# RDG0818/MAZero

Hardware: NVIDIA B200
Metric: mcts_sims_per_sec (higher is better)
Workload: dtype bf16

## Files before the change

### mazero_b200/csrc/search_persist.cuh

```cuda
#pragma once
#include "infer_hmma.cuh"
#include "tree_step.cuh"

namespace maz {
namespace persist {

using namespace hmma;

struct SearchParams {
    Desc d;
    TreeLayout L;
    char *arena;
    const float *lam_pow, *logterm;
    const double *sqrtn;
    int table_len;
    float discount;
    int K, S;
    int *g_err;
    int *idx_y;
    int *greedy_w;
    float *rec_r, *rec_v, *rec_p, *rec_b;
    int *rec_ix, *rec_act;
    long long *tree_clock;
};

__device__ __forceinline__ unsigned long long globaltimer_ns()
{
    unsigned long long t;
    asm volatile("mov.u64 %0, %globaltimer;" : "=l"(t));
    return t;
}

constexpr uint32_t TREE_SCRATCH_OFF = OFF_PH;
constexpr uint32_t TREE_SCRATCH_BYTES = OFF_STAT - OFF_PH;

struct ExtraMap {
    uint32_t hot_stride;
    uint32_t o_qd, o_path, o_exp, o_dep;
    uint32_t o_xr, o_xv, o_xp, o_xb, o_xi, o_xa;
    uint32_t bytes;
};
__host__ __device__ inline uint32_t al16(uint32_t x) { return (x + 15u) & ~15u; }
__host__ __device__ inline ExtraMap extra_map(int rpt, int Nt, int A, int S)
{
    ExtraMap m;
    const uint32_t lv = (uint32_t)S + 2;
    m.o_qd = 64;
    m.o_path = m.o_qd + al16(4 * lv);
    m.o_exp = m.o_path + al16(2 * lv);
    m.o_dep = m.o_exp + al16(2 * lv);
    m.hot_stride = m.o_dep + al16(2 * lv);
    uint32_t o = m.hot_stride * (uint32_t)rpt;
    const uint32_t NA = (uint32_t)Nt * A;
    m.o_xr = o; o += al16(4 * rpt);
    m.o_xv = o; o += al16(4 * rpt);
    m.o_xp = o; o += al16(4 * rpt * NA);
    m.o_xb = o; o += al16(4 * rpt * NA);
    m.o_xi = o; o += al16(4 * rpt);
    m.o_xa = o; o += al16(4 * rpt * Nt);
    m.bytes = o;
    return m;
}
__host__ __device__ inline size_t persist_smem_bytes(int vec_floats, int rpt, int Nt, int A, int S)
{
    return ((smem_bytes(vec_floats) + 15) & ~(size_t)15) + extra_map(rpt, Nt, A, S).bytes;
}

__device__ __forceinline__ void gather_root(const Desc &d, int root, int rl, int ix, const int *tree_act, int lane)
{
    HSM_DECL;
    const int N = d.N;
#pragma unroll 1
    for (int j0 = 0; j0 < N; j0 += 4) {
        float4 v[4];
        int act[4];
#pragma unroll
        for (int u = 0; u < 4; ++u) {
            const int j = j0 + u;
            if (j < N) {
                v[u] = __ldcg(reinterpret_cast<const float4 *>(d.pool + ((size_t)ix * d.B + root) * (size_t)(N * H) + (size_t)j * H) + lane);
                if (d.greedy_pool == nullptr || d.cur < 0) act[u] = tree_act[j];
                else if (j == d.cur) act[u] = tree_act[0];
                else if (j < d.cur) act[u] = d.factor ? __ldcg(d.factor + (size_t)root * N + j) : 0;
                else act[u] = __ldcg(d.greedy_pool + ((size_t)ix * d.B + root) * N + j);
            }
        }
#pragma unroll
        for (int u = 0; u < 4; ++u) {
            const int j = j0 + u;
            if (j < N) {
                const int r = rl * N + j;
                *reinterpret_cast<uint2 *>(hsm + OFF_HH + (size_t)r * LDA + lane * 8) = make_uint2(pack2(v[u].x, v[u].y), pack2(v[u].z, v[u].w));
                if (2 * lane < d.KA)
                    *reinterpret_cast<uint32_t *>(hsm + OFF_ONE + (size_t)r * LDO + lane * 4) =
                        pack2((2 * lane == act[u]) ? 1.f : 0.f, (2 * lane + 1 == act[u]) ? 1.f : 0.f);
            }
        }
    }
}

constexpr int PERSIST_THREADS = NCONS + 128;
constexpr int REGS_COMPUTE = 232, REGS_PRODUCER = 40;

template <bool kProf>
__global__ void __launch_bounds__(PERSIST_THREADS, 1) k_search_persistent(const __grid_constant__ SearchParams P)
{
    HSM_DECL;
    __shared__ __align__(8) uint64_t bar_full[NSLOT], bar_empty[NSLOT], bar_vec;
    const Desc &d = P.d;
    const int tid = threadIdx.x, warp = tid >> 5, lane = tid & 31;

    if (tid == 0) {
        for (int i = 0; i < NSLOT; ++i) { mbar_init(&bar_full[i], 1); mbar_init(&bar_empty[i], NCONS / 32); }
        mbar_init(&bar_vec, 1);
        mbar_fence_init();
    }
    setup_rows(d);
    for (uint32_t o = tid * 16u; o < TM * (uint32_t)LDA + TM * (uint32_t)LDO; o += PERSIST_THREADS * 16u)
        *reinterpret_cast<uint4 *>(hsm + OFF_HH + o) = make_uint4(0u, 0u, 0u, 0u);
    __syncthreads();
    if (warp >= NCONS / 32) {
        asm volatile("setmaxnreg.dec.sync.aligned.u32 %0;" ::"n"(REGS_PRODUCER));
        if (warp == NCONS / 32 && lane == 0) produce_weights(d, bar_full, bar_empty, &bar_vec, P.S);
        return;
    }
    asm volatile("setmaxnreg.inc.sync.aligned.u32 %0;" ::"n"(REGS_COMPUTE));
    Ring ring{bar_full, bar_empty, 0};
    TreeLayout Lprof = P.L;
    if (kProf && P.tree_clock != nullptr)
        Lprof.dbg_clock = P.tree_clock + 2 * P.S + 4 * (long long)gridDim.x + 64 + 4 * (long long)P.d.B;
    const TreeLayout &L = kProf ? Lprof : P.L;
    const int rpt = tile_rpt(d);
    const int root0 = blockIdx.x * rpt;
    const int tree = root0 + warp;
    const bool has_tree = warp < rpt && tree < d.B;
    char *tb = P.arena + (size_t)(has_tree ? tree : 0) * L.slab_bytes;
    const size_t B = (size_t)d.B, NA = (size_t)L.N * L.A;
    const StepScratch scr = carve_step_scratch(reinterpret_cast<char *>(hsm) + TREE_SCRATCH_OFF + (size_t)warp * tree_scratch_bytes(L.N, L.A, L.K, L.S),
                                               L.N, L.A, L.K, L.S);
    const ExtraMap xm = extra_map(rpt, L.N, L.A, L.S);
    char *xbase = reinterpret_cast<char *>(hsm) + ((smem_bytes(d.vec_floats) + 15) & ~(size_t)15);
    char *hb = xbase + (size_t)(warp < rpt ? warp : 0) * xm.hot_stride;
    TreeHdr *hdr = reinterpret_cast<TreeHdr *>(hb);
    const TreeHot hot{reinterpret_cast<uint16_t *>(hb + xm.o_path), reinterpret_cast<float *>(hb + xm.o_qd),
                      reinterpret_cast<uint16_t *>(hb + xm.o_exp), reinterpret_cast<uint16_t *>(hb + xm.o_dep)};
    float *x_r = reinterpret_cast<float *>(xbase + xm.o_xr), *x_v = reinterpret_cast<float *>(xbase + xm.o_xv);
    float *x_p = reinterpret_cast<float *>(xbase + xm.o_xp), *x_b = reinterpret_cast<float *>(xbase + xm.o_xb);
    int *x_i = reinterpret_cast<int *>(xbase + xm.o_xi), *x_a = reinterpret_cast<int *>(xbase + xm.o_xa);
    if (has_tree) {
        const TreeHot g = hot_from_slab(L, tb);
        if (lane < 16) reinterpret_cast<int *>(hdr)[lane] = reinterpret_cast<const int *>(f_hdr(tb))[lane];
        for (int i = lane; i < L.S + 2; i += 32) {
            hot.path[i] = g.path[i]; hot.qd[i] = g.qd[i]; hot.expslot[i] = g.expslot[i]; hot.depth[i] = g.depth[i];
        }
    }
    __syncwarp();

    long long *clk = (kProf && P.tree_clock != nullptr && blockIdx.x == 0 && tid == 0) ? P.tree_clock : nullptr;
    long long *cta_clk = (kProf && P.tree_clock != nullptr && tid == 0) ? P.tree_clock + 2 * P.S + 4 * blockIdx.x : nullptr;
    const long long k0 = cta_clk ? clock64() : 0;
    const unsigned long long g0 = cta_clk ? globaltimer_ns() : 0;
    long long sum_inf = 0, sum_tree = 0;
    long long *tree_clk = (kProf && P.tree_clock != nullptr && has_tree && lane == 0)
                              ? P.tree_clock + 2 * P.S + 4 * (long long)gridDim.x + 64 + 4 * (long long)tree : nullptr;
    long long tc_eb = 0, tc_sel = 0, tc_len = 0, tc_max = 0;

    mbar_wait(&bar_vec, 0);
    setup_head_copies(d);
    cta_sync();

    SimIo io;
    io.idx_x = x_i; io.actions = x_a; io.reward = x_r; io.value = x_v; io.probs = x_p; io.beta = x_b; io.root0 = root0;
    io.logits_out = nullptr;

#pragma unroll 1
    for (int s = 0; s <= P.S; ++s) {
        const long long t1 = cta_clk ? clock64() : 0;
        if (has_tree) {
            const long long q0 = tree_clk ? clock64() : 0;
            if (s > 0) {
                if (P.rec_r != nullptr) {
                    const size_t o = (size_t)(s - 1) * B + tree;
                    if (lane == 0) { P.rec_r[o] = x_r[warp]; P.rec_v[o] = x_v[warp]; }
                    for (int t = lane; t < (int)NA; t += 32) {
                        P.rec_p[o * NA + t] = x_p[(size_t)warp * NA + t];
                        P.rec_b[o * NA + t] = x_b[(size_t)warp * NA + t];
                    }
                }
                expand_backup_device<false>(L, tb, hdr, hot, P.lam_pow, s, P.discount, P.K, x_r + warp, x_v + warp, x_p + (size_t)warp * NA,
                                            x_b + (size_t)warp * NA, scr, lane, P.g_err, kProf ? tree : -1);
            }
            __syncwarp();
            if (kProf && s > 0 && L.dbg_clock != nullptr && tree == 0 && lane == 0) {
                const int order[11] = {0, 1, 2, 11, 12, 13, 14, 15, 3, 4, 5};
                for (int i = 1; i < 11; ++i) L.dbg_clock[16 + i] += L.dbg_clock[order[i]] - L.dbg_clock[order[i - 1]];
            }
            const long long q1 = tree_clk ? clock64() : 0;
            if (s < P.S) {
                select_next_device(L, tb, hdr, hot, P.logterm, P.sqrtn, P.table_len, P.discount, warp, lane, &scr, x_i, nullptr, x_a,
                                   P.g_err);
                __syncwarp();
                const int ix = x_i[warp];
                if (P.rec_ix != nullptr) {
                    const size_t o = (size_t)s * B + tree;
                    if (lane == 0) P.rec_ix[o] = ix;
                    for (int j = lane; j < L.N; j += 32) P.rec_act[o * L.N + j] = x_a[warp * L.N + j];
                }
                gather_root(d, tree, warp, ix, x_a + warp * L.N, lane);
            }
            if (tree_clk) {
                const long long q2 = clock64();
                const int pl = hdr->path_len;
                tc_eb += q1 - q0; tc_sel += q2 - q1; tc_len += pl; tc_max = pl > tc_max ? pl : tc_max;
            }
        }
        cta_sync();
        const long long t2 = cta_clk ? clock64() : 0;
        if (cta_clk) {
            sum_tree += t2 - t1;
            if (clk && s > 0) clk[2 * (s - 1) + 1] = t2 - t1;
        }
        if (s == P.S) break;
        io.next_hidden = d.next_hidden + (size_t)s * B * (size_t)(d.N * H);
        io.greedy = P.greedy_w ? P.greedy_w + (size_t)(s + 1) * B * d.N : nullptr;
        long long *sclk = (clk && s == P.S / 2) ? P.tree_clock + 2 * P.S + 4 * (long long)gridDim.x : nullptr;
        if (sclk) { sclk[0] = t2; sclk[1] = t2; }
        infer_stages(d, io, ring, sclk);
        cta_sync();
        if (cta_clk) {
            const long long t3 = clock64();
            sum_inf += t3 - t2;
            if (clk) clk[2 * s] = t3 - t2;
        }
    }
    if (has_tree && lane < 16) reinterpret_cast<int *>(f_hdr(tb))[lane] = reinterpret_cast<const int *>(hdr)[lane];
    if (tree_clk) { tree_clk[0] = tc_eb; tree_clk[1] = tc_sel; tree_clk[2] = tc_len; tree_clk[3] = tc_max; }
    if (cta_clk) {
        cta_clk[0] = clock64() - k0;
        cta_clk[1] = (long long)(globaltimer_ns() - g0);
        cta_clk[2] = sum_inf;
        cta_clk[3] = sum_tree;
    }
}

}
}
```

### mazero_b200/csrc/tree_step.cuh

```cuda
#pragma once
#include "tree_device.cuh"

namespace maz {

struct LevelAcc {
    unsigned int cnt, nbig;
    unsigned long long minb, maxs;
};
struct StepScratch {
    ExpandScratch ex;
    LevelAcc *acc;
    uint32_t *chase;
    uint16_t *pathc;
};
__host__ __device__ inline size_t tree_scratch_bytes(int N, int A, int K, int S)
{
    const size_t lv = (size_t)S + 2;
    size_t b = expand_scratch_bytes(N, A, K) + lv * sizeof(LevelAcc) + lv * 4 + ((lv * 2 + 15) & ~(size_t)15);
    return (b + 15) & ~(size_t)15;
}
__device__ __forceinline__ StepScratch carve_step_scratch(char *p, int N, int A, int K, int S)
{
    StepScratch s;
    s.ex = carve_scratch(p, N, A);
    p += expand_scratch_bytes(N, A, K);
    s.acc = reinterpret_cast<LevelAcc *>(p);
    p += (size_t)(S + 2) * sizeof(LevelAcc);
    s.chase = reinterpret_cast<uint32_t *>(p);
    p += (size_t)(S + 2) * 4;
    s.pathc = reinterpret_cast<uint16_t *>(p);
    return s;
}

__device__ __forceinline__ float ucb_score_device(const TreeLayout &L, const float *__restrict__ logterm, const double *__restrict__ sqrtn,
                                                  int n, float discount, float pq, float mn, float mx, int mmc, float prior, int cvis,
                                                  float rew, float ws, float wt)
{
    const float pb_c = (L.pbc_dim > 0) ? L.pbc_table[(size_t)n * L.pbc_dim + min(cvis, L.pbc_dim - 1)]
                                       : (float)__dmul_rn((double)logterm[n], __ddiv_rn(sqrtn[n], (double)(cvis + 1)));
    const float prior_score = __fmul_rn(pb_c, prior);
    float v = 0.0f;
    if (cvis != 0) v = __fsub_rn(__fadd_rn(rew, __fmul_rn(discount, __fdiv_rn(ws, wt))), pq);
    if (mmc > 0) {
        const float delta = __fsub_rn(mx, mn);
        const float den = (L.delta_lb < delta) ? delta : L.delta_lb;
        v = __fdiv_rn(__fsub_rn(v, mn), den);
    }
    if (v < 0.0f) v = 0.0f;
    if (v > 1.0f) v = 1.0f;
    return __fadd_rn(prior_score, v);
}

__device__ __forceinline__ void select_path_device(const TreeLayout &L, char *tb, TreeHdr *h, const TreeHot &hot, const float *__restrict__ logterm,
                                                   const double *__restrict__ sqrtn, int table_len, float discount, int tree,
                                                   int lane, int *__restrict__ idx_x, int *__restrict__ idx_y,
                                                   int *__restrict__ act_out, int *g_err)
{
    uint16_t *path = hot.path;
    uint32_t *mt = f_mt(L, tb);

    int mt_pos = h->mt_pos;
    const float mn = h->mm_min, mx = h->mm_max;
    const int mmc = h->mm_cnt;
    const RecRegs root = rec_load(L, tb, 0);
    int C = rec_nchild(root), base = rec_cbase(root), vc = rec_visit(root);
    float pq = rec_pred_value(root);
    constexpr int kPre = 8;
    uint32_t pre = 0;
    if (lane < kPre && mt_pos + lane < kMtN) pre = mt[mt_pos + lane];
    int pre_used = 0;
    const int pre_avail = min(kPre, max(0, kMtN - mt_pos));

    int node = 0, parent_hidx = 0, node_hidx = 0, len = 0, err = 0;
    if (lane == 0) path[0] = 0;
    while (C > 0) {
        float prior = 0.f, rew = 0.f, ws = 0.f, wt = 1.f, cpq = 0.f;
        int cvis = 0, cC = 0, cbase_c = 0, chidx = -1;
        if (lane < C) {
            const RecRegs r = rec_load(L, tb, base + lane);
            prior = rec_prior(r);
            cvis = rec_visit(r);
            rew = rec_reward(r);
            cC = rec_nchild(r);
            cbase_c = rec_cbase(r);
            cpq = rec_pred_value(r);
            chidx = rec_hidx(r);
            ws = rec_wsum(r);
            wt = rec_wtot(r);
        }
        int ci;
        if (node == 0 && vc <= C) {
            ci = vc - 1;
        } else {
            int n = vc - 1;
            if (n >= table_len) n = table_len - 1;
            float score = 0.0f;
            if (lane < C) score = ucb_score_device(L, logterm, sqrtn, n, discount, pq, mn, mx, mmc, prior, cvis, rew, ws, wt);
            const bool valid = (lane < C) && (score > -1000000.0f);
            const uint32_t o = valid ? f2ord(__fadd_rn(score, 0.0f)) : 0u;
            const uint32_t gmax = __reduce_max_sync(MAZ_FULL, o);
            const unsigned anyvalid = __ballot_sync(MAZ_FULL, valid);
            unsigned listmask;
            if (anyvalid) {
                const float M = ord2f(gmax);
                const unsigned ismax = __ballot_sync(MAZ_FULL, valid && score == M);
                const int istar = __ffs(ismax) - 1;
                const float thr = __fsub_rn(M, 0.000001f);
                listmask = __ballot_sync(MAZ_FULL, (lane < C) && (lane > istar) && (score >= thr)) | (1u << istar);
            } else {
                const float thr = __fsub_rn(-1000000.0f, 0.000001f);
                listmask = __ballot_sync(MAZ_FULL, (lane < C) && (score >= thr));
            }
            const int nl = __popc(listmask);
            ci = 0;
            if (nl > 0) {
                uint32_t r;
                if (pre_used < pre_avail) {
                    r = mt_temper(__shfl_sync(MAZ_FULL, pre, pre_used));
                    ++pre_used;
                    ++mt_pos;
                } else {
                    r = mt_next(mt, mt_pos, lane);
                }
                uint32_t mrem = listmask;
                for (uint32_t skip = r % (uint32_t)nl; skip > 0; --skip) mrem &= mrem - 1;
                ci = __ffs(mrem) - 1;
            }
        }
        parent_hidx = node_hidx;
        node = base + ci;
        node_hidx = __shfl_sync(MAZ_FULL, chidx, ci);
        C = __shfl_sync(MAZ_FULL, cC, ci);
        base = __shfl_sync(MAZ_FULL, cbase_c, ci);
        vc = __shfl_sync(MAZ_FULL, cvis, ci);
        pq = __shfl_sync(MAZ_FULL, cpq, ci);
        ++len;
        if (len > L.S + 1) {
            err = kErrPathOverflow;
            break;
        }
        if (lane == 0) path[len] = (uint16_t)node;
    }
    if (lane == 0) {
        h->path_len = len;
        h->mt_pos = mt_pos;
        h->sum_path_len += len;
        idx_x[tree] = parent_hidx;
        if (idx_y) idx_y[tree] = tree;
        if (err) {
            h->err = err;
            *g_err = err;
        }
    }
    const uint8_t *act = f_actions(L, tb) + (size_t)node * L.N;
    for (int j = lane; j < L.N; j += 32) act_out[(size_t)tree * L.N + j] = act[j];
}

static __device__ __noinline__ bool select_path_wide(const TreeLayout &L, char *tb, TreeHdr *h, const TreeHot &hot, const float *__restrict__ logterm,
                                                 const double *__restrict__ sqrtn, int table_len, float discount, int tree, int lane,
                                                 const StepScratch &scr, int *__restrict__ idx_x, int *__restrict__ idx_y,
                                                 int *__restrict__ act_out, int *g_err)
{
    const int n_exp = h->n_expanded, mt_pos = h->mt_pos;
    if (mt_pos + n_exp > kMtN) return false;
    const float mn = h->mm_min, mx = h->mm_max;
    const int mmc = h->mm_cnt;
    const uint32_t *mt = f_mt(L, tb);
    const uint16_t *expslot = hot.expslot;
    const uint16_t *depth = hot.depth;
    const RecRegs root = rec_load(L, tb, 0);
    const int forced = (rec_visit(root) <= rec_nchild(root)) ? 1 : 0;
    constexpr int NPL = 1, CB = 5;
#pragma unroll 1
    for (int e0 = 0; e0 < n_exp; e0 += 32 * NPL) {
        int slot[NPL], C[NPL], base[NPL], n[NPL], dep[NPL];
        float pq[NPL], max_score[NPL];
        unsigned listmask[NPL];
        uint32_t word[NPL];
        bool on[NPL], draw[NPL];
#pragma unroll
        for (int u = 0; u < NPL; ++u) {
            const int e = e0 + 32 * u + lane;
            on[u] = e < n_exp;
            slot[u] = on[u] ? expslot[e] : 0;
            dep[u] = on[u] ? depth[e] : 0;
        }
#pragma unroll
        for (int u = 0; u < NPL; ++u) {
            const int e = e0 + 32 * u + lane;
            const RecRegs nr = rec_load(L, tb, slot[u]);
            C[u] = on[u] ? rec_nchild(nr) : 0;
            base[u] = rec_cbase(nr);
            const int vc = rec_visit(nr);
            pq[u] = rec_pred_value(nr);
            draw[u] = on[u] && !(e == 0 && forced);
            word[u] = draw[u] ? mt[mt_pos + dep[u] - forced] : 0u;
            n[u] = min(vc - 1, table_len - 1);
            max_score[u] = -1000000.0f;
            listmask[u] = 0u;
            if (on[u] && !draw[u]) listmask[u] = 1u << (vc - 1);
        }
        int Cmax = 0;
#pragma unroll
        for (int u = 0; u < NPL; ++u) Cmax = max(Cmax, draw[u] ? C[u] : 0);
#pragma unroll 1
        for (int c0 = 0; c0 < Cmax; c0 += CB) {
            RecRegs r[NPL][CB];
#pragma unroll
            for (int u = 0; u < NPL; ++u)
#pragma unroll
                for (int j = 0; j < CB; ++j)
                    if (draw[u] && c0 + j < C[u]) r[u][j] = rec_load(L, tb, base[u] + c0 + j);
#pragma unroll
            for (int u = 0; u < NPL; ++u)
#pragma unroll
                for (int j = 0; j < CB; ++j)
                    if (draw[u] && c0 + j < C[u]) {
                        const float sc = ucb_score_device(L, logterm, sqrtn, n[u], discount, pq[u], mn, mx, mmc, rec_prior(r[u][j]),
                                                          rec_visit(r[u][j]), rec_reward(r[u][j]), rec_wsum(r[u][j]), rec_wtot(r[u][j]));
                        if (max_score[u] < sc) {
                            max_score[u] = sc;
                            listmask[u] = 1u << (c0 + j);
                        } else if (sc >= __fsub_rn(max_score[u], 0.000001f)) {
                            listmask[u] |= 1u << (c0 + j);
                        }
                    }
        }
#pragma unroll
        for (int u = 0; u < NPL; ++u) {
            if (!on[u]) continue;
            int ci = 0;
            const int nl = __popc(listmask[u]);
            if (nl > 0) {
                uint32_t mrem = listmask[u];
                if (draw[u])
                    for (uint32_t skip = mt_temper(word[u]) % (uint32_t)nl; skip > 0; --skip) mrem &= mrem - 1;
                ci = __ffs(mrem) - 1;
            }
            const int cs = base[u] + ci;
            const RecRegs cr = rec_load(L, tb, cs);
            const int ceid = (rec_nchild(cr) > 0) ? rec_eid(cr) + 1 : 0;
            scr.chase[e0 + 32 * u + lane] = ((uint32_t)cs << 16) | (uint32_t)ceid;
        }
    }
    __syncwarp();
    uint16_t *path = hot.path;
    int e = 0, len = 0, node = 0, parent = 0, err = 0;
    if (lane == 0) path[0] = 0;
    while (true) {
        const uint32_t w = scr.chase[e];
        parent = node;
        node = (int)(w >> 16);
        ++len;
        if (len > L.S + 1) {
            err = kErrPathOverflow;
            break;
        }
        if (lane == 0) path[len] = (uint16_t)node;
        const int ne = (int)(w & 0xffffu);
        if (ne == 0) break;
        e = ne - 1;
    }
    if (lane == 0) {
        h->path_len = len;
        h->mt_pos = mt_pos + len - forced;
        h->sum_path_len += len;
        idx_x[tree] = f_hidx(L, tb)[parent];
        if (idx_y) idx_y[tree] = tree;
        if (err) {
            h->err = err;
            *g_err = err;
        }
    }
    const uint8_t *act = f_actions(L, tb) + (size_t)node * L.N;
    for (int j = lane; j < L.N; j += 32) act_out[(size_t)tree * L.N + j] = act[j];
    return true;
}

__device__ __forceinline__ void select_next_device(const TreeLayout &L, char *tb, TreeHdr *h, const TreeHot &hot, const float *__restrict__ logterm,
                                                   const double *__restrict__ sqrtn, int table_len, float discount, int tree,
                                                   int lane, const StepScratch *scr, int *__restrict__ idx_x, int *__restrict__ idx_y,
                                                   int *__restrict__ act_out, int *g_err)
{
    if (scr != nullptr && h->path_len >= L.wide_min_len &&
        select_path_wide(L, tb, h, hot, logterm, sqrtn, table_len, discount, tree, lane, *scr, idx_x, idx_y, act_out, g_err))
        return;
    select_path_device(L, tb, h, hot, logterm, sqrtn, table_len, discount, tree, lane, idx_x, idx_y, act_out, g_err);
}

constexpr int kLogRegs = 8;

struct LogRegs {
    uint32_t k[kLogRegs];
    float v[kLogRegs];
};
__device__ __forceinline__ void log_prefetch(const TreeLayout &L, char *tb, int log_len0, int lane, LogRegs &lr)
{
    const uint32_t *vk = f_vskey(L, tb);
    const float *vv = f_vsval(L, tb);
#pragma unroll
    for (int c = 0; c < kLogRegs; ++c) {
        const int e = c * 32 + lane;
        lr.k[c] = (e < log_len0) ? vk[e] : 0xffffffffu;
        lr.v[c] = (e < log_len0) ? vv[e] : 0.0f;
    }
}
__device__ __forceinline__ void backup_scatter_entry(const StepScratch &scr, int len, uint32_t k, float v, int e)
{
    const int i = len - (int)((k >> 1) & 0x7fffu);
    if (i >= 0 && scr.pathc[i] == (uint16_t)(k >> 16)) {
        LevelAcc *a = scr.acc + i;
        const unsigned long long oe = ((unsigned long long)f2ord(v) << 32) | (unsigned int)e;
        atomicAdd(&a->cnt, 1u);
        if (k & 1u) {
            atomicAdd(&a->nbig, 1u);
            atomicMin(&a->minb, oe);
        } else {
            atomicMax(&a->maxs, oe);
        }
    }
}

__device__ __forceinline__ void backup_parallel(const TreeLayout &L, char *tb, const TreeHot &hot, const float *__restrict__ lam_pow,
                                                const StepScratch &scr, const LogRegs &lr, int len, int log_len0, int leaf_eid,
                                                float reward_in, float value, float discount, int lane, int &log_len, int &err)
{
    uint32_t *vk = f_vskey(L, tb);
    float *vv = f_vsval(L, tb);
    float *qd = hot.qd;
    const uint16_t *path = hot.path;
    for (int i = lane; i <= len; i += 32) {
        scr.pathc[i] = path[i];
        scr.acc[i].cnt = 0u; scr.acc[i].nbig = 0u; scr.acc[i].minb = ~0ull; scr.acc[i].maxs = 0ull;
    }
    __syncwarp();
#pragma unroll
    for (int c = 0; c < kLogRegs; ++c) backup_scatter_entry(scr, len, lr.k[c], lr.v[c], c * 32 + lane);
    for (int e0 = kLogRegs * 32; e0 < log_len0; e0 += 128) {
        uint32_t k[4];
        float v[4];
#pragma unroll
        for (int u = 0; u < 4; ++u) {
            const int e = e0 + 32 * u + lane;
            k[u] = (e < log_len0) ? vk[e] : 0xffffffffu;
            v[u] = (e < log_len0) ? vv[e] : 0.0f;
        }
#pragma unroll
        for (int u = 0; u < 4; ++u) backup_scatter_entry(scr, len, k[u], v[u], e0 + 32 * u + lane);
    }
    __syncwarp();
    float G = value;
#pragma unroll 1
    for (int base = len; base >= 0; base -= 32) {
        const int nlev = min(32, base + 1);
        const bool active = lane < nlev;
        const int i = base - lane;
        int slot = 0, vis = 0, nh = 0;
        float rew = 0.f, ws = 0.f, wt = 0.f, ppv = 0.f, lp = 0.f;
        if (active) {
            slot = scr.pathc[i];
            lp = lam_pow[len - i];
            if (i == len) {
                rew = reward_in; nh = leaf_eid;
            } else {
                const RecRegs q = rec_load(L, tb, slot);
                rew = rec_reward(q); ws = rec_wsum(q); wt = rec_wtot(q); vis = rec_visit(q); nh = rec_eid(q);
            }
            if (i > 0) ppv = f_pred_value(L, tb)[scr.pathc[i - 1]];
        }
        float myG = 0.f;
        for (int l = 0; l < nlev; ++l) {
            const float r_l = __shfl_sync(MAZ_FULL, rew, l);
            if (lane == l) myG = G;
            G = __fadd_rn(r_l, __fmul_rn(discount, G));
        }
        int myerr = 0;
        if (active) {
            const LevelAcc a = scr.acc[i];
            const uint32_t tag = vs_tag(slot, len - i);
            const VsDecision d = vs_decide(L, (int)a.cnt, (int)a.nbig, (uint32_t)(a.minb >> 32), (int)(uint32_t)a.minb,
                                           (uint32_t)(a.maxs >> 32), (int)(uint32_t)a.maxs, tag, lp, myG, ws, wt);
            myerr = d.err;
            const int pos = log_len + lane;
            if (pos >= L.L) {
                myerr = kErrLogOverflow;
            } else {
                if (d.flip_pos >= 0) vk[d.flip_pos] = d.flip_key;
                vk[pos] = tag | (d.append_big ? 1u : 0u);
                vv[pos] = myG;
            }
            f_visit(L, tb)[slot] = vis + 1;
            f_wsum(L, tb)[slot] = ws;
            f_wtot(L, tb)[slot] = wt;
            if (i != 0) qd[nh] = __fsub_rn(__fadd_rn(rew, __fmul_rn(discount, __fdiv_rn(ws, wt))), ppv);
        }
        const unsigned bad = __ballot_sync(MAZ_FULL, myerr != 0);
        if (bad) err = __shfl_sync(MAZ_FULL, myerr, __ffs(bad) - 1);
        log_len += nlev;
    }
    __syncwarp();
}

__device__ __forceinline__ void minmax_reduce(const TreeHot &hot, int n_expanded, int lane, float &mn, float &mx)
{
    const float *qd = hot.qd;
    uint32_t lo = 0xffffffffu, hi = 0u;
    for (int e = 1 + lane; e < n_expanded; e += 32) {
        const uint32_t o = f2ord(qd[e]);
        lo = min(lo, o);
        hi = max(hi, o);
    }
    mn = ord2f(__reduce_min_sync(MAZ_FULL, lo));
    mx = ord2f(__reduce_max_sync(MAZ_FULL, hi));
}

template <bool kCg = true>
__device__ __forceinline__ void expand_backup_device(const TreeLayout &L, char *tb, TreeHdr *h, const TreeHot &hot, const float *__restrict__ lam_pow,
                                                     int hidx, float discount, int K, const float *__restrict__ reward_ptr,
                                                     const float *__restrict__ value_ptr,
                                                     const float *__restrict__ probs, const float *__restrict__ beta,
                                                     const StepScratch &scr, int lane, int *g_err, int tree = -1)
{
    MAZ_TS(L, tree, lane, 0);
    griddep_launch();
    int tot_nodes = h->tot_nodes, log_len = h->log_len, mt_pos = h->mt_pos, n_expanded = h->n_expanded, err = h->err;
    const int len = h->path_len;
    const int log_len0 = log_len;
    const int leaf_eid = n_expanded;
    MAZ_TS(L, tree, lane, 1);
    LogRegs lr;
    log_prefetch(L, tb, log_len0, lane, lr);
    const int n_draw = (L.A >= 2) ? 2 * K * L.N : 0;
    const bool draws_pre = n_draw > 0 && n_draw <= kMtChunk && mt_pos + n_draw <= kMtN;
    if (draws_pre) {
        const uint32_t *mt = f_mt(L, tb);
        for (int t = lane; t < n_draw; t += 32) scr.ex.draws[t] = mt_temper(mt[mt_pos + t]);
        mt_pos += n_draw;
    }
    const int leaf = hot.path[len];
    MAZ_TS(L, tree, lane, 2);
    griddep_wait();
    const float reward_in = ld_in<kCg>(reward_ptr), value = ld_in<kCg>(value_ptr);
    expand_node<kCg>(L, tb, hot, tot_nodes, n_expanded, mt_pos, err, leaf, hidx, reward_in, value, probs, beta, K, 0.0f, nullptr, scr.ex,
                     lane, draws_pre, tree, true, len);
    MAZ_TS(L, tree, lane, 3);
    backup_parallel(L, tb, hot, lam_pow, scr, lr, len, log_len0, leaf_eid, reward_in, value, discount, lane, log_len, err);
    MAZ_TS(L, tree, lane, 4);
    float mn, mx;
    minmax_reduce(hot, n_expanded, lane, mn, mx);
    if (lane == 0) {
        h->tot_nodes = tot_nodes;
        h->log_len = log_len;
        h->mt_pos = mt_pos;
        h->n_expanded = n_expanded;
        h->mm_cnt = n_expanded - 1;
        h->mm_min = mn;
        h->mm_max = mx;
        h->err = err;
        if (err) *g_err = err;
    }
    MAZ_TS(L, tree, lane, 5);
}

}
```

### profiles/prof_search.py

```python
import os
import sys

import numpy as np
import torch

sys.path.insert(0, os.path.dirname(os.path.dirname(os.path.abspath(__file__))))
from mazero_b200.inference import SmacInference
from mazero_b200.mcts_sampled import SampledMCTS, _DevicePlan, clear_caches
from mazero_b200.synthetic import WORKLOADS, NetworkOutput, SearchConfig, random_state_dict, root_hidden


def main():
    wl = sys.argv[1] if len(sys.argv) > 1 else "3m"
    reps = int(sys.argv[2]) if len(sys.argv) > 2 else 10
    strategies = sys.argv[3:] or ["persistent", "graph"]
    N, A, B, S, K = WORKLOADS[wl]
    B = int(os.environ.get("MAZ_B", B))
    cur = os.environ.get("MAZ_CUR")
    cur = None if cur is None else int(cur)
    dev = torch.device("cuda:0")
    inf = SmacInference(random_state_dict(N, A, seed=0, head_scale=30.0), N, A, device=dev, mode="bf16")
    cfg = SearchConfig(A, S, K)
    flush = torch.empty(256 << 20, dtype=torch.uint8, device=dev)
    for strat in strategies:
        plan = _DevicePlan(inf, B, K, S, cur, cfg, 1.0, strategy=strat)
        times = []
        rpc = max(1, min(8, 32 // N, int(os.environ.get("MAZ_SEARCH_RPT", "8"))))
        ncta = (B + rpc - 1) // rpc
        clk = torch.zeros(2 * S + 4 * ncta + 64 + 4 * B + 32, dtype=torch.int64, device=dev)
        if plan.native is not None and plan.native.strategy == "persistent" and not os.environ.get("MAZ_NO_CLOCK"):
            plan.native.set_debug_clock(clk)
        for r in range(reps + 2):
            h = root_hidden(B, N, seed=r % 5).to(dev)
            pol, vlog = inf.prediction(h)
            val = inf._inv_transform(vlog, inf.vsup).reshape(B, 1)
            plan.stage_roots(h, torch.zeros(B, 1, device=dev), val, pol, None)
            rng = np.random.RandomState(r)
            noise = rng.dirichlet([0.3] * A, B * plan.Nt).astype(np.float32).reshape(B, plan.Nt, A)
            plan.inp_np["noise_raw0"][:] = noise
            plan._stream()
            plan._h2d(0, plan.in_turn[0][1])
            plan._apply_dev_fields()
            flush.zero_()
            e0, e1 = torch.cuda.Event(enable_timing=True), torch.cuda.Event(enable_timing=True)
            e0.record()
            plan._enqueue_search(0, cur, 11 + r, cfg, 0.25, 0)
            e1.record()
            plan.tree.check()
            if r >= 2:
                times.append(e0.elapsed_time(e1))
        t = np.array(times)
        call = clk.cpu().numpy()
        c = call[:2 * S].reshape(S, 2)
        per = call[2 * S:2 * S + 4 * ncta].reshape(-1, 4)
        per = per[per[:, 0] > 0]
        if plan.native is not None and plan.native.strategy == "persistent":
            assert plan.native.roots_per_cta() == rpc, (plan.native.roots_per_cta(), rpc)
        pt = call[2 * S + 4 * ncta + 64:][:4 * B].reshape(B, 4) if len(per) else np.zeros((0, 4))
        if len(pt) and pt[:, 0].any():
            order = np.argsort(-(pt[:, 0] + pt[:, 1]))
            print(f"  per tree (cycles/sim): expand+backup mean {pt[:, 0].mean() / S:.0f} max {pt[:, 0].max() / S:.0f}; select mean "
                  f"{pt[:, 1].mean() / S:.0f} max {pt[:, 1].max() / S:.0f}; mean depth {pt[:, 2].mean() / S:.2f}, max depth {pt[:, 3].max()}")
            print("  slowest trees [expand+backup/sim, select/sim, mean depth, max depth]: " +
                  "; ".join(f"{pt[i, 0] / S:.0f} {pt[i, 1] / S:.0f} {pt[i, 2] / S:.1f} {pt[i, 3]}" for i in order[:6]))
            d = pt[:, 2] / S
            for lo, hi in ((0, 2), (2, 3), (3, 5), (5, 8), (8, 100)):
                m = (d >= lo) & (d < hi)
                if m.any():
                    print(f"    mean depth in [{lo},{hi}): {m.sum()} trees, expand+backup {pt[m, 0].mean() / S:.0f}, select {pt[m, 1].mean() / S:.0f} cycles/sim")
        ts = call[2 * S + 4 * ncta + 64 + 4 * B:][:32]
        if ts[:6].all():
            nm = {0: "start", 1: "header", 2: "prefetch issued", 11: "beta/probs staged", 12: "cdf", 13: "sampled", 14: "keys merged",
                  15: "children", 3: "expansion done", 4: "backup", 5: "minmax+header"}
            order = [0, 1, 2, 11, 12, 13, 14, 15, 3, 4, 5]
            print("  tree 0, phase cycles per simulation (mean over the search): " +
                  ", ".join(f"{nm[b]} {ts[16 + i + 1] / S:.0f}" for i, b in enumerate(order[1:])))
        st_all = call[2 * S + 4 * ncta:][:64]
        hs = st_all[40:]
        hs = hs[hs > 0]
        if len(hs) > 2:
            print("  heads2 phases (cycles): " + " ".join(str(int(v)) for v in np.diff(hs)))
        st = st_all[:40]
        st = st[st > 0]
        if len(st) > 2:
            names = ["gather", "sync", "inproj"] + [f"L{l}.{x}" for l in range(3) for x in ("qkv", "attn", "out+ln", "lin1", "lin2+ln")] + \
                    ["-", "dynamics", "heads1", "heads2"]
            dl = np.diff(st)
            print("  stage cycles (CTA 0, middle simulation): " + ", ".join(f"{n} {int(v)}" for n, v in zip(names, dl)))
        if len(per):
            ghz = per[:, 0] / np.maximum(per[:, 1], 1)
            print(f"  {len(per)} CTAs: total cycles mean {per[:, 0].mean():.0f} min {per[:, 0].min()} max {per[:, 0].max()}; "
                  f"ns mean {per[:, 1].mean():.0f} max {per[:, 1].max()}; SM clock {ghz.mean():.3f} GHz; "
                  f"inference cycles/sim mean {per[:, 2].mean() / S:.0f} max {per[:, 2].max() / S:.0f}; "
                  f"tree cycles/sim mean {per[:, 3].mean() / S:.0f} min {per[:, 3].min() / S:.0f} max {per[:, 3].max() / S:.0f}")
        print(f"{wl} B={B} cur={cur} strategy={strat} ({plan.native.strategy if plan.native else 'legacy'}): "
              f"{t.mean():.3f} ms/search (min {t.min():.3f} max {t.max():.3f}) -> {B * S / t.mean() / 1e3:.2f} M root-sims/s"
              + (f"; CTA0 cycles/sim: inference {c[:, 0].mean():.0f} tree {c[:, 1].mean():.0f}" if c.any() else ""))
        out = {k: v.clone() for k, v in plan.turn_out[0].items()}
        plan.close()
        del plan
    clear_caches()


if __name__ == "__main__":
    main()
```

Measured before the change: 18.21 million.

## Stage tree backup log scan, RNG draws and minmax in helper warps during inference

Three idle warps left over from the producer warpgroup now run a helper loop. While the consumer warps run network inference, the helpers precompute each tree's backup log scatter into per-level accumulators, the tempered Mersenne Twister draws, and the off-path min/max of Q values, all stored in a new shared-memory TreeStage. The next expand/backup step consumes these staged results and only merges the min/max over the updated path nodes. The full-CTA barriers become named barriers that include the helpers. In exchange, each tree uses more shared memory and the synchronisation gets more complex, and trees whose path is longer than 32 levels fall back to the original path.

```diff
diff --git a/mazero_b200/csrc/search_persist.cuh b/mazero_b200/csrc/search_persist.cuh
--- a/mazero_b200/csrc/search_persist.cuh
+++ b/mazero_b200/csrc/search_persist.cuh
@@ -38,6 +38,7 @@
     uint32_t hot_stride;
     uint32_t o_qd, o_path, o_exp, o_dep;
     uint32_t o_xr, o_xv, o_xp, o_xb, o_xi, o_xa;
+    uint32_t o_stage;
     uint32_t bytes;
 };
 __host__ __device__ inline uint32_t al16(uint32_t x) { return (x + 15u) & ~15u; }
@@ -58,6 +59,7 @@
     m.o_xb = o; o += al16(4 * rpt * NA);
     m.o_xi = o; o += al16(4 * rpt);
     m.o_xa = o; o += al16(4 * rpt * Nt);
+    m.o_stage = o; o += (uint32_t)sizeof(TreeStage) * rpt;
     m.bytes = o;
     return m;
 }
@@ -101,6 +103,43 @@
 
 constexpr int PERSIST_THREADS = NCONS + 128;
 constexpr int REGS_COMPUTE = 232, REGS_PRODUCER = 40;
+constexpr int HELPER_WARP0 = NCONS / 32 + 1, N_HELPERS = 3;
+constexpr int BAR_TREES_DONE = 2;
+constexpr int BAR_STAGED = 3;
+constexpr int BAR_HELPER_THREADS = NCONS + 32 * N_HELPERS;
+
+__device__ __forceinline__ TreeStage *stage_of(const Desc &d, const TreeLayout &L, int rpt, int t)
+{
+    HSM_DECL;
+    return reinterpret_cast<TreeStage *>(hsm + ((smem_bytes(d.vec_floats) + 15) & ~(size_t)15) + extra_map(rpt, L.N, L.A, L.S).o_stage) + t;
+}
+
+__device__ __forceinline__ void named_bar_arrive(int id, int nthreads)
+{
+    asm volatile("bar.arrive %0, %1;" ::"r"(id), "r"(nthreads) : "memory");
+}
+
+static __device__ __noinline__ void helper_loop(const SearchParams &P, int helper, int lane)
+{
+    HSM_DECL;
+    const Desc &d = P.d;
+    const int rpt = tile_rpt(d), root0 = blockIdx.x * rpt;
+    const ExtraMap xm = extra_map(rpt, P.L.N, P.L.A, P.L.S);
+    char *xbase = reinterpret_cast<char *>(hsm) + ((smem_bytes(d.vec_floats) + 15) & ~(size_t)15);
+    TreeStage *stage = reinterpret_cast<TreeStage *>(xbase + xm.o_stage);
+#pragma unroll 1
+    for (int s = 0; s < P.S; ++s) {
+        named_bar_sync(BAR_TREES_DONE, BAR_HELPER_THREADS);
+#pragma unroll 1
+        for (int t = helper; t < rpt && root0 + t < d.B; t += N_HELPERS) {
+            char *hb = xbase + (size_t)t * xm.hot_stride;
+            const TreeHot hot{reinterpret_cast<uint16_t *>(hb + xm.o_path), reinterpret_cast<float *>(hb + xm.o_qd),
+                              reinterpret_cast<uint16_t *>(hb + xm.o_exp), reinterpret_cast<uint16_t *>(hb + xm.o_dep)};
+            stage_step(P.L, P.arena + (size_t)(root0 + t) * P.L.slab_bytes, reinterpret_cast<const TreeHdr *>(hb), hot, P.K, stage + t, lane);
+        }
+        named_bar_arrive(BAR_STAGED, BAR_HELPER_THREADS);
+    }
+}
 
 template <bool kProf>
 __global__ void __launch_bounds__(PERSIST_THREADS, 1) k_search_persistent(const __grid_constant__ SearchParams P)
@@ -121,7 +160,11 @@
     __syncthreads();
     if (warp >= NCONS / 32) {
         asm volatile("setmaxnreg.dec.sync.aligned.u32 %0;" ::"n"(REGS_PRODUCER));
-        if (warp == NCONS / 32 && lane == 0) produce_weights(d, bar_full, bar_empty, &bar_vec, P.S);
+        if (warp == NCONS / 32) {
+            if (lane == 0) produce_weights(d, bar_full, bar_empty, &bar_vec, P.S);
+        } else {
+            helper_loop(P, warp - HELPER_WARP0, lane);
+        }
         return;
     }
     asm volatile("setmaxnreg.inc.sync.aligned.u32 %0;" ::"n"(REGS_COMPUTE));
@@ -188,12 +231,13 @@
                     }
                 }
                 expand_backup_device<false>(L, tb, hdr, hot, P.lam_pow, s, P.discount, P.K, x_r + warp, x_v + warp, x_p + (size_t)warp * NA,
-                                            x_b + (size_t)warp * NA, scr, lane, P.g_err, kProf ? tree : -1);
+                                            x_b + (size_t)warp * NA, scr, lane, P.g_err, kProf ? tree : -1,
+                                            stage_of(d, L, rpt, warp));
             }
             __syncwarp();
             if (kProf && s > 0 && L.dbg_clock != nullptr && tree == 0 && lane == 0) {
-                const int order[11] = {0, 1, 2, 11, 12, 13, 14, 15, 3, 4, 5};
-                for (int i = 1; i < 11; ++i) L.dbg_clock[16 + i] += L.dbg_clock[order[i]] - L.dbg_clock[order[i - 1]];
+                const int order[12] = {0, 1, 2, 11, 12, 13, 14, 15, 3, 7, 4, 5};
+                for (int i = 1; i < 12; ++i) L.dbg_clock[16 + i] += L.dbg_clock[order[i]] - L.dbg_clock[order[i - 1]];
             }
             const long long q1 = tree_clk ? clock64() : 0;
             if (s < P.S) {
@@ -214,7 +258,8 @@
                 tc_eb += q1 - q0; tc_sel += q2 - q1; tc_len += pl; tc_max = pl > tc_max ? pl : tc_max;
             }
         }
-        cta_sync();
+        if (s < P.S) named_bar_sync(BAR_TREES_DONE, BAR_HELPER_THREADS);
+        else cta_sync();
         const long long t2 = cta_clk ? clock64() : 0;
         if (cta_clk) {
             sum_tree += t2 - t1;
@@ -226,7 +271,7 @@
         long long *sclk = (clk && s == P.S / 2) ? P.tree_clock + 2 * P.S + 4 * (long long)gridDim.x : nullptr;
         if (sclk) { sclk[0] = t2; sclk[1] = t2; }
         infer_stages(d, io, ring, sclk);
-        cta_sync();
+        named_bar_sync(BAR_STAGED, BAR_HELPER_THREADS);
         if (cta_clk) {
             const long long t3 = clock64();
             sum_inf += t3 - t2;
diff --git a/mazero_b200/csrc/tree_step.cuh b/mazero_b200/csrc/tree_step.cuh
--- a/mazero_b200/csrc/tree_step.cuh
+++ b/mazero_b200/csrc/tree_step.cuh
@@ -305,11 +305,11 @@
         lr.v[c] = (e < log_len0) ? vv[e] : 0.0f;
     }
 }
-__device__ __forceinline__ void backup_scatter_entry(const StepScratch &scr, int len, uint32_t k, float v, int e)
+__device__ __forceinline__ void backup_scatter_entry(LevelAcc *acc, const uint16_t *pathc, int len, uint32_t k, float v, int e)
 {
     const int i = len - (int)((k >> 1) & 0x7fffu);
-    if (i >= 0 && scr.pathc[i] == (uint16_t)(k >> 16)) {
-        LevelAcc *a = scr.acc + i;
+    if (i >= 0 && pathc[i] == (uint16_t)(k >> 16)) {
+        LevelAcc *a = acc + i;
         const unsigned long long oe = ((unsigned long long)f2ord(v) << 32) | (unsigned int)e;
         atomicAdd(&a->cnt, 1u);
         if (k & 1u) {
@@ -321,35 +321,97 @@
     }
 }
 
+constexpr int kStageLv = 32;
+enum : int { kStagedLog = 1, kStagedDraws = 2, kStagedMinmax = 4 };
+struct TreeStage {
+    LevelAcc acc[kStageLv];
+    uint32_t draws[kMtChunk];
+    uint32_t mm_lo, mm_hi;
+    int flags;
+    int pad;
+};
+static_assert(sizeof(TreeStage) % 16 == 0, "TreeStage keeps 16-byte alignment in arrays");
+
+__device__ __forceinline__ void stage_step(const TreeLayout &L, char *tb, const TreeHdr *h, const TreeHot &hot, int K,
+                                           TreeStage *st, int lane)
+{
+    const int len = h->path_len, log_len0 = h->log_len, mt_pos = h->mt_pos, n_exp = h->n_expanded;
+    int flags = kStagedMinmax;
+    if (len < kStageLv) {
+        if (lane <= len) { st->acc[lane].cnt = 0u; st->acc[lane].nbig = 0u; st->acc[lane].minb = ~0ull; st->acc[lane].maxs = 0ull; }
+        __syncwarp();
+        const uint32_t *vk = f_vskey(L, tb);
+        const float *vv = f_vsval(L, tb);
+#pragma unroll 1
+        for (int e0 = 0; e0 < log_len0; e0 += 64) {
+            uint32_t k[2];
+            float v[2];
+#pragma unroll
+            for (int u = 0; u < 2; ++u) {
+                const int e = e0 + 32 * u + lane;
+                k[u] = (e < log_len0) ? __ldcg(vk + e) : 0xffffffffu;
+                v[u] = (e < log_len0) ? __ldcg(vv + e) : 0.0f;
+            }
+#pragma unroll
+            for (int u = 0; u < 2; ++u) backup_scatter_entry(st->acc, hot.path, len, k[u], v[u], e0 + 32 * u + lane);
+        }
+        flags |= kStagedLog;
+    }
+    const int n_draw = (L.A >= 2) ? 2 * K * L.N : 0;
+    if (n_draw > 0 && n_draw <= kMtChunk && mt_pos + n_draw <= kMtN) {
+        const uint32_t *mt = f_mt(L, tb);
+        for (int t = lane; t < n_draw; t += 32) st->draws[t] = mt_temper(__ldcg(mt + mt_pos + t));
+        flags |= kStagedDraws;
+    }
+    uint32_t lo = 0xffffffffu, hi = 0u;
+    for (int e = 1 + lane; e < n_exp; e += 32) {
+        const int dep = hot.depth[e];
+        if (dep <= len && hot.path[dep] == hot.expslot[e]) continue;
+        const uint32_t o = f2ord(hot.qd[e]);
+        lo = min(lo, o);
+        hi = max(hi, o);
+    }
+    lo = __reduce_min_sync(MAZ_FULL, lo);
+    hi = __reduce_max_sync(MAZ_FULL, hi);
+    if (lane == 0) { st->mm_lo = lo; st->mm_hi = hi; st->flags = flags; }
+}
+
 __device__ __forceinline__ void backup_parallel(const TreeLayout &L, char *tb, const TreeHot &hot, const float *__restrict__ lam_pow,
                                                 const StepScratch &scr, const LogRegs &lr, int len, int log_len0, int leaf_eid,
-                                                float reward_in, float value, float discount, int lane, int &log_len, int &err)
+                                                float reward_in, float value, float discount, int lane, int &log_len, int &err,
+                                                int tree = -1, const LevelAcc *sacc = nullptr, uint32_t *mm = nullptr)
 {
     uint32_t *vk = f_vskey(L, tb);
     float *vv = f_vsval(L, tb);
     float *qd = hot.qd;
     const uint16_t *path = hot.path;
-    for (int i = lane; i <= len; i += 32) {
-        scr.pathc[i] = path[i];
-        scr.acc[i].cnt = 0u; scr.acc[i].nbig = 0u; scr.acc[i].minb = ~0ull; scr.acc[i].maxs = 0ull;
-    }
-    __syncwarp();
-#pragma unroll
-    for (int c = 0; c < kLogRegs; ++c) backup_scatter_entry(scr, len, lr.k[c], lr.v[c], c * 32 + lane);
-    for (int e0 = kLogRegs * 32; e0 < log_len0; e0 += 128) {
-        uint32_t k[4];
-        float v[4];
-#pragma unroll
-        for (int u = 0; u < 4; ++u) {
-            const int e = e0 + 32 * u + lane;
-            k[u] = (e < log_len0) ? vk[e] : 0xffffffffu;
-            v[u] = (e < log_len0) ? vv[e] : 0.0f;
-        }
-#pragma unroll
-        for (int u = 0; u < 4; ++u) backup_scatter_entry(scr, len, k[u], v[u], e0 + 32 * u + lane);
-    }
-    __syncwarp();
+    const LevelAcc *acc = sacc ? sacc : scr.acc;
+    const uint16_t *pathc = sacc ? path : scr.pathc;
+    if (sacc == nullptr) {
+        for (int i = lane; i <= len; i += 32) {
+            scr.pathc[i] = path[i];
+            scr.acc[i].cnt = 0u; scr.acc[i].nbig = 0u; scr.acc[i].minb = ~0ull; scr.acc[i].maxs = 0ull;
+        }
+        __syncwarp();
+#pragma unroll
+        for (int c = 0; c < kLogRegs; ++c) backup_scatter_entry(scr.acc, scr.pathc, len, lr.k[c], lr.v[c], c * 32 + lane);
+        for (int e0 = kLogRegs * 32; e0 < log_len0; e0 += 128) {
+            uint32_t k[4];
+            float v[4];
+#pragma unroll
+            for (int u = 0; u < 4; ++u) {
+                const int e = e0 + 32 * u + lane;
+                k[u] = (e < log_len0) ? vk[e] : 0xffffffffu;
+                v[u] = (e < log_len0) ? vv[e] : 0.0f;
+            }
+#pragma unroll
+            for (int u = 0; u < 4; ++u) backup_scatter_entry(scr.acc, scr.pathc, len, k[u], v[u], e0 + 32 * u + lane);
+        }
+        __syncwarp();
+    }
+    MAZ_TS(L, tree, lane, 7);
     float G = value;
+    uint32_t mlo = 0xffffffffu, mhi = 0u;
 #pragma unroll 1
     for (int base = len; base >= 0; base -= 32) {
         const int nlev = min(32, base + 1);
@@ -358,7 +420,7 @@
         int slot = 0, vis = 0, nh = 0;
         float rew = 0.f, ws = 0.f, wt = 0.f, ppv = 0.f, lp = 0.f;
         if (active) {
-            slot = scr.pathc[i];
+            slot = pathc[i];
             lp = lam_pow[len - i];
             if (i == len) {
                 rew = reward_in; nh = leaf_eid;
@@ -366,7 +428,7 @@
                 const RecRegs q = rec_load(L, tb, slot);
                 rew = rec_reward(q); ws = rec_wsum(q); wt = rec_wtot(q); vis = rec_visit(q); nh = rec_eid(q);
             }
-            if (i > 0) ppv = f_pred_value(L, tb)[scr.pathc[i - 1]];
+            if (i > 0) ppv = f_pred_value(L, tb)[pathc[i - 1]];
         }
         float myG = 0.f;
         for (int l = 0; l < nlev; ++l) {
@@ -376,7 +438,7 @@
         }
         int myerr = 0;
         if (active) {
-            const LevelAcc a = scr.acc[i];
+            const LevelAcc a = acc[i];
             const uint32_t tag = vs_tag(slot, len - i);
             const VsDecision d = vs_decide(L, (int)a.cnt, (int)a.nbig, (uint32_t)(a.minb >> 32), (int)(uint32_t)a.minb,
                                            (uint32_t)(a.maxs >> 32), (int)(uint32_t)a.maxs, tag, lp, myG, ws, wt);
@@ -392,12 +454,17 @@
             f_visit(L, tb)[slot] = vis + 1;
             f_wsum(L, tb)[slot] = ws;
             f_wtot(L, tb)[slot] = wt;
-            if (i != 0) qd[nh] = __fsub_rn(__fadd_rn(rew, __fmul_rn(discount, __fdiv_rn(ws, wt))), ppv);
+            if (i != 0) {
+                const float q = __fsub_rn(__fadd_rn(rew, __fmul_rn(discount, __fdiv_rn(ws, wt))), ppv);
+                qd[nh] = q;
+                if (mm) { mlo = min(mlo, f2ord(q)); mhi = max(mhi, f2ord(q)); }
+            }
         }
         const unsigned bad = __ballot_sync(MAZ_FULL, myerr != 0);
         if (bad) err = __shfl_sync(MAZ_FULL, myerr, __ffs(bad) - 1);
         log_len += nlev;
     }
+    if (mm) { mm[0] = __reduce_min_sync(MAZ_FULL, mlo); mm[1] = __reduce_max_sync(MAZ_FULL, mhi); }
     __syncwarp();
 }
 
@@ -419,7 +486,8 @@
                                                      int hidx, float discount, int K, const float *__restrict__ reward_ptr,
                                                      const float *__restrict__ value_ptr,
                                                      const float *__restrict__ probs, const float *__restrict__ beta,
-                                                     const StepScratch &scr, int lane, int *g_err, int tree = -1)
+                                                     const StepScratch &scr, int lane, int *g_err, int tree = -1,
+                                                     const TreeStage *stg = nullptr)
 {
     MAZ_TS(L, tree, lane, 0);
     griddep_launch();
@@ -428,26 +496,40 @@
     const int log_len0 = log_len;
     const int leaf_eid = n_expanded;
     MAZ_TS(L, tree, lane, 1);
+    const int staged = stg ? stg->flags : 0;
     LogRegs lr;
-    log_prefetch(L, tb, log_len0, lane, lr);
+    if (!(staged & kStagedLog)) log_prefetch(L, tb, log_len0, lane, lr);
     const int n_draw = (L.A >= 2) ? 2 * K * L.N : 0;
     const bool draws_pre = n_draw > 0 && n_draw <= kMtChunk && mt_pos + n_draw <= kMtN;
+    ExpandScratch ex = scr.ex;
     if (draws_pre) {
-        const uint32_t *mt = f_mt(L, tb);
-        for (int t = lane; t < n_draw; t += 32) scr.ex.draws[t] = mt_temper(mt[mt_pos + t]);
+        if (staged & kStagedDraws) {
+            ex.draws = const_cast<uint32_t *>(stg->draws);
+        } else {
+            const uint32_t *mt = f_mt(L, tb);
+            for (int t = lane; t < n_draw; t += 32) ex.draws[t] = mt_temper(mt[mt_pos + t]);
+        }
         mt_pos += n_draw;
     }
     const int leaf = hot.path[len];
     MAZ_TS(L, tree, lane, 2);
     griddep_wait();
     const float reward_in = ld_in<kCg>(reward_ptr), value = ld_in<kCg>(value_ptr);
-    expand_node<kCg>(L, tb, hot, tot_nodes, n_expanded, mt_pos, err, leaf, hidx, reward_in, value, probs, beta, K, 0.0f, nullptr, scr.ex,
+    expand_node<kCg>(L, tb, hot, tot_nodes, n_expanded, mt_pos, err, leaf, hidx, reward_in, value, probs, beta, K, 0.0f, nullptr, ex,
                      lane, draws_pre, tree, true, len);
     MAZ_TS(L, tree, lane, 3);
-    backup_parallel(L, tb, hot, lam_pow, scr, lr, len, log_len0, leaf_eid, reward_in, value, discount, lane, log_len, err);
+    uint32_t mm[2];
+    const int staged_b = stg ? stg->flags : 0;
+    backup_parallel(L, tb, hot, lam_pow, scr, lr, len, log_len0, leaf_eid, reward_in, value, discount, lane, log_len, err, tree,
+                    (staged_b & kStagedLog) ? stg->acc : nullptr, (staged_b & kStagedMinmax) ? mm : nullptr);
     MAZ_TS(L, tree, lane, 4);
     float mn, mx;
-    minmax_reduce(hot, n_expanded, lane, mn, mx);
+    if ((staged_b & kStagedMinmax) && n_expanded == leaf_eid + 1) {
+        mn = ord2f(min(stg->mm_lo, mm[0]));
+        mx = ord2f(max(stg->mm_hi, mm[1]));
+    } else {
+        minmax_reduce(hot, n_expanded, lane, mn, mx);
+    }
     if (lane == 0) {
         h->tot_nodes = tot_nodes;
         h->log_len = log_len;
diff --git a/profiles/prof_search.py b/profiles/prof_search.py
--- a/profiles/prof_search.py
+++ b/profiles/prof_search.py
@@ -71,8 +71,8 @@
         ts = call[2 * S + 4 * ncta + 64 + 4 * B:][:32]
         if ts[:6].all():
             nm = {0: "start", 1: "header", 2: "prefetch issued", 11: "beta/probs staged", 12: "cdf", 13: "sampled", 14: "keys merged",
-                  15: "children", 3: "expansion done", 4: "backup", 5: "minmax+header"}
-            order = [0, 1, 2, 11, 12, 13, 14, 15, 3, 4, 5]
+                  15: "children", 3: "expansion done", 7: "backup log pass", 4: "backup level update", 5: "minmax+header"}
+            order = [0, 1, 2, 11, 12, 13, 14, 15, 3, 7, 4, 5]
             print("  tree 0, phase cycles per simulation (mean over the search): " +
                   ", ".join(f"{nm[b]} {ts[16 + i + 1] / S:.0f}" for i, b in enumerate(order[1:])))
         st_all = call[2 * S + 4 * ncta:][:64]
```

Result: faster. 18.46 million, median of 6 (+1.4%).
